# kyotovision-public/DRMNet

Measured on AMD Instinct MI355X. Metric: U-Net denoise steps/sec on 3x128x256 refmaps, higher is better.
Workload: dtype emulated fp32: f16 hi*hi + e4m3 cross terms (~15-bit products), fp32 acc; 1e-4 contract

## Files before the change

drmnet_amd/_lib.py:

```python
from __future__ import annotations

import ctypes as C
import os
from typing import Optional, Sequence

import torch

_HERE = os.path.dirname(os.path.abspath(__file__))
LIB_PATH = os.environ.get("DRM_LIB_PATH") or os.path.join(_HERE, "csrc", "libdrmnet_hip.so")
ABI_VERSION = 3
MAX_LEVELS = 8
LOSS_WORKSPACE_BYTES = 2048
DIFFUSION_LOSS_MAX_PARTS = 32


def diffusion_loss_workspace_bytes(B: int) -> int:
    return int(B) * DIFFUSION_LOSS_MAX_PARTS * 2 * 8


SYMBOLS = [
    "drm_abi_version", "drm_last_error",
    "drm_unet_create", "drm_unet_destroy", "drm_unet_param_count", "drm_unet_param_info", "drm_unet_load_params",
    "drm_unet_workspace_bytes", "drm_unet_forward",
    "drm_linear_forward", "drm_timestep_embedding", "drm_op_norm_act_conv", "drm_op_resblock", "drm_op_attention_block",
    "drm_drmnet_create", "drm_drmnet_destroy", "drm_drmnet_workspace_bytes", "drm_drmnet_set_batch_parts", "drm_drmnet_set_batch_part_min", "drm_drmnet_step", "drm_drmnet_sample",
    "drm_sampler_workspace_bytes", "drm_ddim_sample", "drm_ddim_sample_logged", "drm_ddpm_sample", "drm_ddim_sample_ex", "drm_ddpm_sample_ex", "drm_randn",
    "drm_profile_enable", "drm_profile_reset", "drm_profile_collect", "drm_unet_set_precision", "drm_set_op_precision",
    "drm_refmap_workspace_bytes", "drm_refmap_mask_make", "drm_erode_mask",
    "drm_unet_load_params_set", "drm_unet_use_set", "drm_set_graph_replay", "drm_set_upconv_split", "drm_graph_launches",
    "drm_map_chain", "drm_masked_log_range", "drm_luminance_scale", "drm_mirmap2envmap", "drm_hdr2ldr", "drm_resize", "drm_profile_variants",
    "drm_render_refmap", "drm_brdf_eval", "drm_render_refmap_views", "drm_validation_losses",
    "drm_render_refmap_lit", "drm_render_light_workspace_bytes",
    "drm_render_mesh_workspace_bytes", "drm_render_mesh",
    "drm_mesh_bvh_bytes", "drm_mesh_bvh_build", "drm_mesh_occluded", "drm_render_mesh_shadowed", "drm_render_mesh_lit",
    "drm_mesh_closest_hit", "drm_render_mesh_bounced",
    "drm_render_normals", "drm_image_from_refmap",
    "drm_obs_forward_process", "drm_diffusion_losses",
]


class UNetDesc(C.Structure):
    _fields_ = [
        ("kind", C.c_int32), ("in_channels", C.c_int32), ("model_channels", C.c_int32), ("out_channels", C.c_int32),
        ("num_res_blocks", C.c_int32), ("n_levels", C.c_int32), ("channel_mult", C.c_int32 * MAX_LEVELS),
# ... 116 lines not shown
    L.drm_ddpm_sample_ex.argtypes = [vp, fp, fp, fp, C.POINTER(C.c_float), i32, i32, fp, C.c_uint64, C.POINTER(SamplerOptions), i32, i32, i32, vp, C.c_size_t, vp]
    L.drm_randn.argtypes = [fp, C.c_size_t, C.c_uint64, C.c_uint64, vp]
    u8p = vp
    L.drm_refmap_workspace_bytes.argtypes = [C.c_int64, i32, C.c_float]
    L.drm_refmap_workspace_bytes.restype = C.c_size_t
    L.drm_refmap_mask_make.argtypes = [fp, fp, C.c_int64, i32, i32, C.c_float, i32, fp, u8p, vp, C.c_size_t, vp]
    L.drm_erode_mask.argtypes = [u8p, i32, i32, i32, u8p, vp]
    L.drm_unet_set_precision.argtypes = [vp, i32]
    L.drm_set_op_precision.argtypes = [i32]
    L.drm_profile_enable.argtypes = [i32]
    L.drm_profile_enable.restype = None
    L.drm_profile_reset.restype = None
    L.drm_profile_collect.argtypes = [C.POINTER(C.c_double), C.POINTER(C.c_double), C.POINTER(C.c_double), C.POINTER(C.c_int64)]
    L.drm_set_graph_replay.argtypes = [i32]
    L.drm_set_upconv_split.argtypes = [i32]
    L.drm_graph_launches.restype = C.c_int64
    L.drm_map_chain.argtypes = [fp, fp, C.c_int64, i32, C.POINTER(C.c_int32), C.POINTER(C.c_float), i32, fp, fp, fp, vp]
    L.drm_masked_log_range.argtypes = [fp, fp, i32, i32, i32, fp, fp, vp]
    L.drm_luminance_scale.argtypes = [fp, i32, i32, C.c_float, fp, vp]
    L.drm_mirmap2envmap.argtypes = [fp, fp, fp, i32, i32, i32, i32, i32, i32, i32, i32, vp]
    L.drm_hdr2ldr.argtypes = [fp, u8p, i32, C.c_float, C.c_float, fp, vp]
    L.drm_resize.argtypes = [fp, fp, i32, i32, i32, i32, i32, i32, vp]
    L.drm_profile_variants.argtypes = [C.c_char_p, C.c_size_t]
    L.drm_profile_variants.restype = C.c_size_t
    L.drm_render_refmap.argtypes = [fp, fp, fp, i32, i32, i32, i32, i32, i32, i32, vp]
    L.drm_brdf_eval.argtypes = [fp, i32, fp, fp, fp, fp, C.c_int64, vp]
    L.drm_render_refmap_views.argtypes = [fp, i32, fp, fp, fp, i32, i32, i32, i32, i32, i32, i32, vp]
    L.drm_render_refmap_lit.argtypes = [fp, i32, fp, fp, fp, i32, i32, i32, i32, i32, i32, i32, i32, vp, C.c_size_t, vp]
    L.drm_render_light_workspace_bytes.argtypes = [i32, i32, i32, i32]
    L.drm_render_light_workspace_bytes.restype = C.c_size_t
# ... 68 lines not shown
```

drmnet_amd/csrc/abi.hip:

```cpp
#include <atomic>
#include <cstring>
#include <memory>

#include "bvh.h"
#include "profiler.h"
#include "samplers.h"

using namespace drm;

struct drm_unet {
  UNet net;
};
struct drm_drmnet {
  DrmnetSampler s;
};

namespace {

int make_arena(Arena& ar, void* ws, size_t bytes, size_t need) {
  if (need == 0) return DRM_ERR_INVALID;
  if (bytes < need || ws == nullptr) {
    set_error("workspace too small: need " + std::to_string(need) + " bytes, got " + std::to_string(bytes));
    return DRM_ERR_WORKSPACE;
  }
// ... 409 lines not shown
    DRM_REQUIRE(precision_valid(precision),
                "precision must be 0 (fp32 MFMA), 1 (split fp16 x3), 2 (plain fp16 operands), 3 (split fp16 with fp8 cross terms) or 4 (plain bf16 operands)");
    g_op_precision.store(precision, std::memory_order_relaxed);
    return DRM_OK;
  });
}

int drm_set_upconv_split(int mode) {
  return guarded([&]() -> int {
    DRM_REQUIRE(mode >= 0 && mode <= 2, "upconv split mode: 0 = never, 1 = by the measured rule, 2 = wherever the form applies");
    set_upconv_split(mode);
    return DRM_OK;
  });
}

int drm_set_graph_replay(int on) {
  set_graph_replay(on != 0);
  return DRM_OK;
}
int64_t drm_graph_launches(void) { return (int64_t)graph_launches(); }

void drm_profile_enable(int on) { prof_enable(on); }
void drm_profile_reset(void) { prof_reset(); }
int drm_profile_collect(double* ms, double* flops, double* bytes, int64_t* launches) {
  return guarded([&]() -> int {
    DRM_REQUIRE(ms && flops && bytes && launches, "null argument");
    prof_collect(ms, flops, bytes, launches);
    return DRM_OK;
  });
}
// ... 220 lines not shown
```

drmnet_amd/csrc/common.h:

```cpp
#pragma once
#include <hip/hip_runtime.h>
#include <stdint.h>
#include <stdio.h>
#include <atomic>
#include <string>
#include "conv_forms.h"
#include "gn_fold.h"

namespace drm {

void set_error(const std::string& msg);
const char* last_error();

#define DRM_OK 0
#define DRM_ERR_INVALID 1
#define DRM_ERR_HIP 2
#define DRM_ERR_WORKSPACE 3
#define DRM_ERR_STATE 4

#define DRM_HIP_CHECK(expr)                                                                              \
  do {                                                                                                   \
    hipError_t _e = (expr);                                                                              \
    if (_e != hipSuccess) {                                                                              \
      ::drm::set_error(std::string(#expr) + " failed: " + hipGetErrorString(_e) + " at " + __FILE__ + ":" + \
// ... 66 lines not shown
  int terms = 3;
  int mx_site = 0;
#ifdef DRM_S2_STAMP
  unsigned* stamp_out = nullptr;
  int stamp_block = 0, stamp_tile0 = 0;
#endif
  double2* stat_out = nullptr;
  float* pool_out = nullptr;
  double2* pool_stat = nullptr;
  const float* w_inv_scale = nullptr;
  int ld0 = 0;
  int gn_ld = 0;
  long long w_img_stride_f4 = 0;
  const float* w_inv_img = nullptr;
  int prof_kind = -1;
  const float* in_inv = nullptr;
  GnFold gnf;
};
struct ConvWork { double flops, bytes; };
inline ConvWork conv_work(const ConvArgs& a, int taps) {
  const double cin = a.cin_real > 0 ? a.cin_real : (a.C0 + a.C1), cout = a.out_nchw ? a.cout_valid : a.Cout;
  const double px = (double)a.N * a.H * a.W;
  const double px_in = (double)a.N * ((a.H >> a.up0) * (a.W >> a.up0)) * a.C0 + px * a.C1;
  return {2.0 * px * (taps == 4 ? 9 : taps) * cin * cout, 4.0 * (px_in + px * cout * (a.res ? 2 : 1) + (double)taps * cin * cout)};
}
enum ConvKernel : unsigned char { CONV_NONE, CONV_IGEMM, CONV_PIPELINE };
enum SplitFinish : unsigned char { SPLIT_NONE, SPLIT_IN_LAUNCH, SPLIT_REDUCE };
struct ConvPlan {
  ConvKernel kernel = CONV_NONE;
  int terms = 0;
  ConvTile tile = TILE_128x32;
  int th = 0, tw = 0;
  bool ragged = false;
  int kc = 32;
  int ksplit = 1;
  SplitFinish finish = SPLIT_NONE;
  size_t tickets = 0;
  bool pool = false;
  bool gn_fold = false;
// ... 2 lines not shown
ConvPlan plan_conv(const ConvArgs& a, int precision, bool want_pool = false, bool gn_foldable = false);
bool conv_split_weights(int precision, int cin);
int launch_conv(const ConvArgs& a, const ConvPlan& p, hipStream_t s);
template <int TAPS, int TERMS> int dispatch_s2(const ConvArgs& a, const ConvPlan& p, hipStream_t s);
int no_form(const ConvPlan& p);
size_t packed_conv_weight_split_floats(int taps, int CoutP, int CinP);
int launch_pack_conv_weight_split(const float* w, float* packed, float* scales, unsigned* scratch, int Cout, int Cin, int taps, int CoutP,
                                  int CinP, hipStream_t s, bool mx = false, bool bf16 = false);
enum Precision { PREC_FP32 = 0, PREC_F16X3 = 1, PREC_F16 = 2, PREC_F16MX = 3, PREC_BF16 = 4 };
inline bool precision_valid(int p) { return p >= PREC_FP32 && p <= PREC_BF16; }
inline int precision_terms(int p) { return p == PREC_F16 ? 1 : (p == PREC_BF16 ? 4 : (p == PREC_FP32 ? 0 : 3)); }
int launch_pack_conv_weight(const float* w, float* packed, int Cout, int Cin, int taps, int CoutP, int CinP, hipStream_t s);
int pack_conv_image(int precision, const float* w, float* packed, float* scale, unsigned* scratch, int Cout, int Cin, int taps, int CoutP, int CinP,
                    bool mx_site, hipStream_t s);
int launch_fold_upconv_weight(const float* w, float* wa, float* wb, int Cout, int C0, int C1, hipStream_t s);
int launch_fold_attn_params(const float* qkv_w, const float* qkv_b, const float* proj_w, const float* proj_b, float* w_out, float* b_out, int C,
                            hipStream_t s);
size_t packed_conv_weight_floats(int taps, int CoutP, int CinP);

int launch_chan_moments(const float* x, int N, int HW, int C, double* partial , double2* mom , hipStream_t s);
int chan_moments_splits(int HW, int C);
int launch_act_pow2_scale(const double2* mom0, int C0, int lo0, int hi0, double cnt0, const double2* mom1, int C1, double cnt1,
                          const unsigned* absmax_bits, int Ctab, int N, float* scale, float* shift, float* inv, hipStream_t s, int absmax_parts = 1);
int launch_gn_finalize(const double2* mom0, int C0, double inv0, const double2* mom1, int C1, double inv1, const float* gamma,
                       const float* beta, int N, float* scale, float* shift, hipStream_t s, double cnt0 = 0.0, double cnt1 = 0.0,
                       float* guard_scale = nullptr, float* guard_shift = nullptr, float* guard_inv = nullptr);

size_t refmap_workspace_bytes(long long n, int res, float thr);
int launch_refmap_mask_make(const float* colors, const float* normals, long long n, int C, int res, float thr, int min_points, float* refmap,
                            unsigned char* refmask, void* ws, size_t ws_bytes, hipStream_t s);
// ... 106 lines not shown
```

drmnet_amd/csrc/conv.hip:

```cpp

#include "common.h"
#include "profiler.h"

namespace drm {

typedef float f32x16 __attribute__((ext_vector_type(16)));

template <int TAPS, int TH, int TW, int WM, int WN, int MT, int NT, int KC>
struct Cfg {
  static constexpr int BM = WM * MT * 32;
  static constexpr int BN = WN * NT * 32;
  static constexpr int TN = BM / (TH * TW);
  static constexpr int HALO = (TAPS == 9) ? 1 : 0;
  static constexpr int HT = TH + 2 * HALO, WT = TW + 2 * HALO;
  static constexpr int HPI = HT * WT;
  static constexpr int HP = TN * HPI;
  static constexpr int KG = KC / 4;
  static constexpr int TPI = 256 / TN;
  static constexpr int A_SLOTS = (HPI * KG + TPI - 1) / TPI;
  static constexpr int B_F4 = KG * BN;
  static constexpr int B_SLOTS = (B_F4 + 255) / 256;
  static constexpr int LDS_F4 = KG * HP + 2 * B_F4;
  static_assert(BM == 128 && WM * WN == 4, "4 waves, 128 GEMM rows");
  static_assert(KG % 2 == 0 && TPI % KG == 0, "k-group split across lane halves");
// ... 302 lines not shown
        *d = make_double2(d->x + a, d->y + c2);
      }
    }
  }
}

#define DRM_X(TAPS, TERMS) extern template int dispatch_s2<TAPS, TERMS>(const ConvArgs&, const ConvPlan&, hipStream_t);
DRM_S2_UNITS(DRM_X)
#undef DRM_X
int launch_conv(const ConvArgs& a, const ConvPlan& p, hipStream_t s) {
  DRM_REQUIRE(a.taps == 9 || a.taps == 1 || a.taps == 4, "conv taps must be 9, 1 or 4 (the parity form of a 3x3 over a nearest-x2 input)");
  DRM_REQUIRE(a.taps != 4 || (p.kernel == CONV_PIPELINE && p.finish == SPLIT_NONE), "the parity (4-tap) form runs on the pipeline kernel, un-split");
  DRM_REQUIRE(a.N > 0 && a.H > 0 && a.W > 0, "conv shape");
  DRM_REQUIRE(!a.up0 || (a.H % 2 == 0 && a.W % 2 == 0), "upsampled source needs even output size");
  DRM_REQUIRE(a.ksplit == p.ksplit && (p.ksplit == 1 || a.split_ws), "split-K launch without its slab workspace");
  if (p.kernel == CONV_IGEMM) return launch_igemm(a, p, s);
  DRM_REQUIRE(p.kernel == CONV_PIPELINE, "no conv kernel takes this shape (per-image weights: split modes, maps of whole 16x16 tiles, 128-channel multiples)");
  DRM_REQUIRE(a.Cout % 32 == 0 && (a.C0 + a.C1) % 32 == 0 && a.C0 % 32 == 0, "split conv needs channels % 32 == 0");
  DRM_REQUIRE(a.terms == p.terms, "ConvArgs::terms differs from the plan");
  DRM_REQUIRE(p.terms != 2 || (a.taps != 1 && a.gn_scale && !a.in_inv && a.w_img_stride_f4 == 0), "f16mx: 3x3 convs on a GroupNorm-ed input only");
  auto run = [&](const ConvArgs& x) -> int {
#define DRM_X(TAPS, TERMS) if (a.taps == TAPS && p.terms == TERMS) return dispatch_s2<TAPS, TERMS>(x, p, s);
    DRM_S2_UNITS(DRM_X)
#undef DRM_X
    return no_form(p);
  };
  if (p.finish != SPLIT_REDUCE) return run(a);
  ConvArgs part = a;
  part.out = a.split_ws;
  part.split_ws = nullptr;
// ... 38 lines not shown
```

drmnet_amd/csrc/conv_split.hip:

```cpp
#include "common.h"
#include "profiler.h"

namespace drm {

__global__ void absmax_kernel(const float* __restrict__ w, size_t n, unsigned* __restrict__ out_bits) {
  float m = 0.f;
  for (size_t i = blockIdx.x * (size_t)blockDim.x + threadIdx.x; i < n; i += (size_t)gridDim.x * blockDim.x) m = fmaxf(m, fabsf(w[i]));
#pragma unroll
  for (int o = 32; o > 0; o >>= 1) m = fmaxf(m, __shfl_xor(m, o));
  if ((threadIdx.x & 63) == 0) atomicMax(out_bits, __float_as_uint(m));
}

__global__ void split_scale_kernel(const unsigned* __restrict__ absmax_bits, float* __restrict__ scales) {
  const float m = __uint_as_float(*absmax_bits);
  int k = 0;
  if (m > 0.f && m < INFINITY) {
    int e;
    frexpf(m, &e);
    k = 14 - e;
    if (k > 30) k = 30;
    if (k < -30) k = -30;
  }
  scales[0] = ldexpf(1.0f, k);
  scales[1] = ldexpf(1.0f, -k);
// ... 128 lines not shown
      const int ci = t % C1;
      const int co = (int)(t / C1);
      wb[k] = w[((size_t)co * Cin + C0 + ci) * 9 + tap];
    }
  }
}

int launch_fold_upconv_weight(const float* w, float* wa, float* wb, int Cout, int C0, int C1, hipStream_t s) {
  DRM_REQUIRE(w && wa && wb && Cout > 0 && C0 > 0 && C1 > 0, "upsampled-conv weight fold: arguments");
  const size_t n = (size_t)16 * Cout * C0 + (size_t)Cout * C1 * 9;
  hipLaunchKernelGGL(fold_upconv_weight_kernel, dim3((unsigned)std::min<size_t>((n + 255) / 256, 4096)), dim3(256), 0, s, w, wa, wb, Cout, C0, C1);
  DRM_HIP_CHECK(hipGetLastError());
  return DRM_OK;
}

}
```

drmnet_amd/csrc/conv_split2.hip:

```cpp
#include <algorithm>
#include <utility>
#include <vector>
#include <cstdio>
#include <string>

#include "common.h"
#include "conv_epilogue.h"
#include "profiler.h"

#ifdef DRM_S2_STAMP
#define S2_STAMP(id)                                                                               \
  do {                                                                                             \
    if (stamp_on && stamp_n < 120) {                                                               \
      unsigned long long t_;                                                                       \
      __builtin_amdgcn_sched_barrier(0);                                                           \
      asm volatile("s_memtime %0\n\ts_waitcnt lgkmcnt(0)" : "=s"(t_)::"memory");                   \
      __builtin_amdgcn_sched_barrier(0);                                                           \
      if (lane == 0) {                                                                             \
        stamp_lds[(wave * 120 + stamp_n) * 2] = (unsigned)(id);                                    \
        stamp_lds[(wave * 120 + stamp_n) * 2 + 1] = (unsigned)t_;                                  \
      }                                                                                            \
      ++stamp_n;                                                                                   \
    }                                                                                              \
  } while (0)
// ... 203 lines not shown
  bool stamp_on = false;
  if (a.stamp_out && (int)blockIdx.x == (a.stamp_block & 0xFFFF))
    for (int k = tid; k < C::NW * 240; k += C::NTHR) stamp_lds[k] = 0;
  stamp_on = a.stamp_out && (int)blockIdx.x == (a.stamp_block & 0xFFFF) && a.stamp_tile0 == 0;
  S2_STAMP(60);
#endif

  const int Ctot = a.C0 + a.C1;
  const int nch_all = Ctot / C::KC;
  const int ks = a.ksplit > 1 ? a.ksplit : 1;
  const int split = blockIdx.y;
  const int chunk0 = split * nch_all / ks;
  const int nchunks = (split + 1) * nch_all / ks - chunk0;
  const int NGT = nchunks * C::NG;
  constexpr bool FUSE = SK;
  static_assert(!SK || (WM == 4 && WN == 1 && MT == 1 && NT == 1 && !RAG), "split-K launches use the 128-row x 32-channel tiles (plan_conv)");
  const bool fused = FUSE && ks > 1 && a.split_ws != nullptr;
  float* const out_s = (fused ? a.split_ws : a.out) + (size_t)split * a.split_stride;
  const bool has_gn = a.gn_scale != nullptr;

  const int l_img = tid / C::TPI;
  const int l_tid = tid % C::TPI;
  const int l_o = tid % C::OCT;
  f32x4 areg[C::A_SLOTS][2];
  f32x4 sc[2], sh[2];
  unsigned avalid = 0;

  auto load_A_piece = [&](const TilePos& tp, int chunk, int piece) {
    const int c = (chunk0 + chunk) * C::KC;
    const float* src;
// ... 596 lines not shown
        }
        S2_STAMP(20 + 4 * (i * NT + c));
        const bool first = ks == 1;
        const float bias = (a.bias && first) ? a.bias[co] : 0.f;
        float rv[16], ev[4], sv[4];
#pragma unroll
        for (int g = 0; g < 4; ++g) {
          ev[g] = (a.emb && first) ? a.emb[(size_t)nimg[g] * a.emb_stride + co] : 0.f;
          sv[g] = epi_scale(a, nimg[g], inv_scale);
        }
#ifdef DRM_S2_STAMP
        const bool abl_noload = a.stamp_block & 0x200000;
#else
        constexpr bool abl_noload = false;
#endif
        if (a.res && first && !abl_noload) {
#pragma unroll
          for (int e = 0; e < 16; ++e) rv[e] = a.res[(pixb[e >> 2] + (e & 3)) * a.Cout + co];
        } else {
#pragma unroll
          for (int e = 0; e < 16; ++e) rv[e] = 0.f;
        }
        float s0 = 0.f, q0 = 0.f, s1 = 0.f, q1 = 0.f;
        float v[16];
#pragma unroll
        for (int e = 0; e < 16; ++e) {
          const int g = e >> 2;
          v[e] = epi_value(acc[i][c][e] * sv[g], bias, ev[g], rv[e]);
          acc[i][c][e] = 0.f;
#ifdef DRM_S2_STAMP
          if (a.stamp_block & 0x100000) continue;
// ... 259 lines not shown
  if (a.stamp_out && (int)blockIdx.x == (a.stamp_block & 0xFFFF)) {
    asm volatile("s_waitcnt lgkmcnt(0)" ::: "memory");
    __builtin_amdgcn_s_barrier();
    for (int k = tid; k < C::NW * 240; k += C::NTHR) a.stamp_out[k] = stamp_lds[k];
  }
#endif
}

template <int TAPS, int TH, int TW, int WM, int WN, int MT, int NT, int R, int TPS, int TERMS = 3, bool RAG = false, bool SK = false, bool POOL = false>
static int launch_s2(const ConvArgs& a, hipStream_t s) {
  using C = S2Cfg<TAPS, TH, TW, WM, WN, MT, NT, R, TPS, TERMS>;
  constexpr auto kern = conv_split2_kernel<TAPS, TH, TW, WM, WN, MT, NT, R, TPS, TERMS, RAG, SK, POOL>;
  DRM_REQUIRE(RAG || (a.H % TH == 0 && a.W % TW == 0), "conv tile does not divide the map");
  DRM_REQUIRE(POOL == (a.pool_out != nullptr), "pooled output: only launches plan_conv pools");
  DRM_REQUIRE(!POOL || (a.pool_stat && a.stat_out && a.ksplit <= 1 && !a.out_nchw), "pooled output: needs both statistics tables, no split-K");
  if constexpr (TAPS == 4) {
    static_assert(!RAG && !SK && !POOL, "the parity form has no ragged, split-K or pooled instantiation");
    DRM_REQUIRE(!a.bias && !a.emb && !a.res && !a.stat_out && !a.out_nchw && a.ksplit <= 1 && !a.gnf.mom0 && !a.in_inv && a.w_img_stride_f4 == 0,
                "parity (4-tap) conv: weight un-scaling only -- no bias, emb, residual, statistics, split-K or GroupNorm fold");
    DRM_REQUIRE(a.C1 == 0 && !a.up0 && a.Cout % 4 == 0 && (a.Cout / 4) % C::BN == 0, "parity (4-tap) conv: one stored source, a Cout tile inside one parity");
  }
  const size_t lds_bytes = (size_t)(C::LDS_F4 + (POOL ? C::ST_F4 : 0)) * sizeof(float4);
  static_assert((C::LDS_F4 + (POOL ? C::ST_F4 : 0)) * 16 <= 160 * 1024, "LDS budget");
  const DeviceInfo* di = device_info();
  if (!di) return DRM_ERR_STATE;
  DRM_TRY(opt_in_lds<kern>(lds_bytes, di));
  const int groups = (a.N + C::TN - 1) / C::TN;
  const long long tiles = (long long)groups * ((a.H + TH - 1) / TH) * ((a.W + TW - 1) / TW) * (a.Cout / C::BN);
  DRM_REQUIRE(tiles > 0 && tiles < (1ll << 31), "conv grid size");
  const int per_cu = std::max(1, std::min((int)(di->lds_per_cu / lds_bytes), 8 / C::NW));
// ... 94 lines not shown
```

drmnet_amd/csrc/engine.h:

```cpp
#pragma once
#include <map>
#include <string>
#include <tuple>
#include <vector>

#include "../../include/drmnet_hip.h"
#include "common.h"

namespace drm {

struct Arena {
  char* base = nullptr;
  size_t cap = 0, off = 0, peak = 0;
  bool dry = false;
  bool failed = false;
  void* alloc_bytes(size_t bytes) {
    const size_t a = (off + 255) & ~size_t(255);
    off = a + bytes;
    if (off > peak) peak = off;
    if (dry) return nullptr;
    if (off > cap) {
      failed = true;
      return nullptr;
    }
// ... 63 lines not shown
  size_t scale_dst = 0;
  bool mx_site = false;
  bool attn_fold = false;
  int up_c0 = 0;
  size_t upa_dst = 0, upa_scale = 0, upb_dst = 0, upb_scale = 0;
};

struct ResLayer {
  int cin = 0, cout = 0;
  size_t n1_w = 0, n1_b = 0, c1_w = 0, c1_b = 0, n2_w = 0, n2_b = 0, c2_w = 0, c2_b = 0, sk_w = 0, sk_b = 0;
  size_t c1_s = 0, c2_s = 0, sk_s = 0;
  int emb_off = 0;
  bool has_skip = false;
  int up_c0 = 0;
  size_t c1a_w = 0, c1a_s = 0, c1b_w = 0, c1b_s = 0;
};
struct AttnLayer {
  int ch = 0;
  size_t n_w = 0, n_b = 0, qkv_w = 0, qkv_b = 0, qkv_s = 0;
};
struct Layer {
  enum Kind { RES, ATTN, DOWN, UP } kind;
  ResLayer res;
  AttnLayer attn;
};

struct ParamTable {
  std::vector<ParamSlot> params;
  int emb_dim = 0, emb_total = 0;
  size_t wbuf_floats = 0;
// ... 34 lines not shown
  int dry_forward(int N, int H, int W, Arena& probe);
  ~UNet();
};

struct Ctx {
  Arena* ar;
  hipStream_t s;
  int N;
  int precision = PREC_FP32;
  bool dry() const { return ar->dry; }
  bool split() const { return precision == PREC_F16X3 || precision == PREC_F16 || precision == PREC_F16MX || precision == PREC_BF16; }
  int terms() const { return precision_terms(precision); }
};
Act new_act(Ctx& c, int C, int H, int W);
void set_upconv_split(int mode);
inline bool upconv_split_packable(int c0, int c1, int cout) { return c0 > 0 && c1 > 0 && c0 % 32 == 0 && c1 % 32 == 0 && cout % 32 == 0; }
int ensure_moments(Ctx& c, Act& a);
int expect_raw_sums(Ctx& c, Act& a);
int run_resblock(Ctx& c, const float* wbuf, const ResLayer& r, Act& x0, Act* x1, const float* emb_all, int emb_stride, Act& out, Act* pool = nullptr,
                 bool* pooled = nullptr);
int run_attention(Ctx& c, const float* wbuf, const AttnLayer& a, Act& x, Act& out);
int run_conv(Ctx& c, ConvArgs& a, const ConvPlan& p, const float* wbuf, size_t scale_off, Act* stats_for = nullptr);
int raw_input_guard(Ctx& c, ConvArgs& a, const ConvPlan& p, Act* x0, int lo0, int hi0, Act* x1, const unsigned* absmax_bits, int Ctab, int absmax_parts = 1);
int gn_params(Ctx& c, Act& x0, Act* x1, const float* gamma, const float* beta, float* scale, float* shift, ConvArgs* guard_for = nullptr,
              ConvArgs* fold_into = nullptr);

}
```

drmnet_amd/csrc/engine.hip:

```cpp
#include "engine.h"

#include <algorithm>
#include <atomic>
#include <deque>
#include <mutex>

namespace drm {

static thread_local std::string g_err;
void set_error(const std::string& msg) { g_err = msg; }
const char* last_error() { return g_err.c_str(); }

const DeviceInfo* device_info() {
  constexpr int MAX_DEV = 64;
  static DeviceInfo info[MAX_DEV];
  static std::atomic<int> state[MAX_DEV];
  int dev = 0;
  if (hipGetDevice(&dev) != hipSuccess || dev < 0 || dev >= MAX_DEV) {
    set_error("device_info: no current HIP device");
    return nullptr;
  }
  int st = state[dev].load(std::memory_order_acquire);
  if (st == 0) {
    static std::mutex mu;
// ... 81 lines not shown
    p.upb_scale = r.c1b_s = reserve(64);
  }
  r.c1_b = add_copy(px + ".in_layers.2.bias", {cout});
  r.emb_off = emb_total;
  emb_total += cout;
  ParamSlot ew; ew.name = px + ".emb_layers.1.weight"; ew.shape = {cout, emb_dim}; ew.kind = PK_COPY; ew.count = (size_t)cout * emb_dim; ew.dst = (size_t)-1; ew.cout = r.emb_off;
  params.push_back(ew);
  ParamSlot eb; eb.name = px + ".emb_layers.1.bias"; eb.shape = {cout}; eb.kind = PK_COPY; eb.count = (size_t)cout; eb.dst = (size_t)-2; eb.cout = r.emb_off;
  params.push_back(eb);
  r.n2_w = add_copy(px + ".out_layers.0.weight", {cout});
  r.n2_b = add_copy(px + ".out_layers.0.bias", {cout});
  r.c2_w = add_conv(px + ".out_layers.3.weight", cout, cout, 3, cout, cout, false, &r.c2_s, true);
  r.c2_b = add_copy(px + ".out_layers.3.bias", {cout});
  if (r.has_skip) {
    r.sk_w = add_conv(px + ".skip_connection.weight", cout, cin, 1, cout, cin, false, &r.sk_s);
    r.sk_b = add_copy(px + ".skip_connection.bias", {cout});
  }
}

void ParamTable::add_attn(Layer& l, const std::string& px, int ch) {
  l.kind = Layer::ATTN;
  AttnLayer& a = l.attn;
  a.ch = ch;
  a.n_w = add_copy(px + ".norm.weight", {ch});
  a.n_b = add_copy(px + ".norm.bias", {ch});
  a.qkv_w = add_conv(px + ".qkv.weight", 3 * ch, ch, 1, 3 * ch, ch, true, &a.qkv_s);
  params.back().attn_fold = true;
  a.qkv_b = add_copy(px + ".qkv.bias", {3 * ch});
  params.back().kind = PK_FOLDED;
  ParamSlot pw; pw.name = px + ".proj_out.weight"; pw.shape = {ch, ch, 1}; pw.kind = PK_FOLDED; pw.count = (size_t)ch * ch;
// ... 114 lines not shown
  }
}

int pack_conv_image(int precision, const float* w, float* packed, float* scale, unsigned* scratch, int Cout, int Cin, int taps, int CoutP, int CinP,
                    bool mx_site, hipStream_t s) {
  if (conv_split_weights(precision, CinP))
    return launch_pack_conv_weight_split(w, packed, scale, scratch, Cout, Cin, taps, CoutP, CinP, s, precision == PREC_F16MX && mx_site,
                                         precision == PREC_BF16);
  return launch_pack_conv_weight(w, packed, Cout, Cin, taps, CoutP, CinP, s);
}

size_t ParamTable::staging_floats() const {
  size_t n = 0;
  for (const ParamSlot& p : params) {
    if (p.attn_fold) n = std::max(n, (size_t)p.cout * p.cin + (size_t)p.cout);
    if (p.up_c0) n = std::max(n, (size_t)16 * p.cout * p.up_c0 + (size_t)9 * p.cout * (p.cin - p.up_c0));
  }
  return n;
}

int ParamTable::pack(const float* const* ptrs, int count, float* wbuf, int precision, float* staging, hipStream_t s) const {
  DRM_REQUIRE(count == (int)params.size(), "parameter count mismatch: got " + std::to_string(count) + ", expected " + std::to_string(params.size()));
  DRM_HIP_CHECK(hipMemsetAsync(wbuf, 0, wbuf_floats * sizeof(float), s));
  auto conv = [&](const float* w, size_t dst, size_t scale_dst, int cout, int cin, int taps, int coutp, int cinp, bool mx_site) -> int {
    return pack_conv_image(precision, w, wbuf + dst, wbuf + scale_dst, reinterpret_cast<unsigned*>(wbuf + scratch_off), cout, cin, taps, coutp, cinp,
                           mx_site, s);
  };
  for (size_t i = 0; i < params.size(); ++i) {
    const ParamSlot& p = params[i];
    DRM_REQUIRE(ptrs[i] != nullptr, "null parameter pointer for " + p.name);
    if (p.kind == PK_FOLDED) continue;
    const float* w = ptrs[i];
    if (p.attn_fold) {
      DRM_REQUIRE(i + 3 < params.size() && ptrs[i + 1] && ptrs[i + 2] && ptrs[i + 3], "attention block parameters of " + p.name);
      float* fb = staging + (size_t)p.cout * p.cin;
      DRM_TRY(launch_fold_attn_params(ptrs[i], ptrs[i + 1], ptrs[i + 2], ptrs[i + 3], staging, fb, p.cin, s));
      DRM_HIP_CHECK(hipMemcpyAsync(wbuf + params[i + 1].dst, fb, (size_t)p.cout * sizeof(float), hipMemcpyDeviceToDevice, s));
      w = staging;
    }
    if (p.kind == PK_COPY) {
      DRM_HIP_CHECK(hipMemcpyAsync(wbuf + p.dst, w, p.count * sizeof(float), hipMemcpyDeviceToDevice, s));
    } else {
      DRM_TRY(conv(w, p.dst, p.scale_dst, p.cout, p.cin, p.taps, p.coutp, p.cinp, p.mx_site));
      if (p.up_c0) {
        const int c0 = p.up_c0, c1 = p.cin - p.up_c0;
        float* wa = staging;
        float* wb = staging + (size_t)16 * p.cout * c0;
        DRM_TRY(launch_fold_upconv_weight(w, wa, wb, p.cout, c0, c1, s));
        DRM_TRY(conv(wa, p.upa_dst, p.upa_scale, 4 * p.cout, c0, 4, 4 * p.cout, c0, p.mx_site));
        DRM_TRY(conv(wb, p.upb_dst, p.upb_scale, p.cout, c1, 9, p.cout, c1, p.mx_site));
      }
    }
  }
  return DRM_OK;
}

int UNet::load(const float* const* ptrs, int count, hipStream_t s, int set) {
  DRM_REQUIRE(set >= 0 && set < NSETS, "weight set index");
  if (!wsets[set]) DRM_HIP_CHECK(hipMalloc(reinterpret_cast<void**>(&wsets[set]), wbuf_floats * sizeof(float)));
// ... 117 lines not shown
  ConvPlan p4, p9;
};
static UpconvSplit plan_upconv_split(const Ctx& c, const ResLayer& r, const ConvArgs& a, const ConvPlan& pa, const Act& x0, const Act* x1) {
  UpconvSplit u;
  const int mode = g_upconv_split.load(std::memory_order_relaxed);
  if (mode == 0 || !r.up_c0 || !x0.up || !x1 || x0.C != r.up_c0 || !upconv_split_packable(x0.C, x1->C, r.cout)) return u;
  auto plain = [](const ConvPlan& p) { return p.kernel == CONV_PIPELINE && !p.ragged && p.ksplit == 1 && !p.gn_fold && !p.pool; };
  if (!plain(pa)) return u;
  u.a4.C0 = x0.C; u.a4.N = a.N; u.a4.H = a.H >> 1; u.a4.W = a.W >> 1; u.a4.taps = 4; u.a4.Cout = 4 * r.cout; u.a4.mx_site = 1;
  u.b9.C0 = x1->C; u.b9.N = a.N; u.b9.H = a.H; u.b9.W = a.W; u.b9.taps = 9; u.b9.Cout = r.cout; u.b9.mx_site = 1;
  u.p4 = plan_conv(u.a4, c.precision);
  u.p9 = plan_conv(u.b9, c.precision);
  if (!plain(u.p4) || !plain(u.p9)) return u;
  if (r.cout % tile_shape(u.p4.tile).bn() != 0) return u;
  if (mode == 1 && (u.p4.tile > TILE_256x128 || u.p9.tile > TILE_256x128)) return u;
  u.on = true;
  return u;
}

int run_resblock(Ctx& c, const float* Wb, const ResLayer& r, Act& x0, Act* x1, const float* emb_all, int emb_stride, Act& out, Act* pool, bool* pooled) {
  DRM_TRY(arena_ok(c));
  const int H = x0.H, W = x0.W;
  const int C0 = x0.C, C1 = x1 ? x1->C : 0;
  DRM_REQUIRE(C0 + C1 == r.cin, "resblock input channels");
  DRM_REQUIRE(!x1 || (x1->H == H && x1->W == W && !x1->up), "resblock skip tensor shape");
  DRM_REQUIRE(r.has_skip || (!x1 && !x0.up), "identity skip on a concatenated / upsampled input is not supported");
  const size_t mark = c.ar->mark();
  float* sc1 = c.ar->alloc<float>((size_t)c.N * r.cin);
  float* sh1 = c.ar->alloc<float>((size_t)c.N * r.cin);
  Act h1 = new_act(c, r.cout, H, W);
  float* sc2 = c.ar->alloc<float>((size_t)c.N * r.cout);
  float* sh2 = c.ar->alloc<float>((size_t)c.N * r.cout);
  ConvArgs k;
  ConvArgs a;
  a.src0 = x0.p; a.src1 = x1 ? x1->p : nullptr; a.C0 = C0; a.C1 = C1; a.up0 = x0.up;
  a.N = c.N; a.H = H; a.W = W; a.taps = 9; a.Cout = r.cout; a.mx_site = 1;
  const ConvPlan pa = plan_conv(a, c.precision, false, true);
  ConvPlan pk;
  if (r.has_skip) {
    k.C0 = C0; k.C1 = C1; k.N = c.N; k.H = H; k.W = W; k.taps = 1; k.Cout = r.cout;
    pk = plan_conv(k, c.precision);
  }
  DRM_TRY(gn_params(c, x0, x1, Wb + r.n1_w, Wb + r.n1_b, sc1, sh1, pk.split() ? &k : nullptr, pa.gn_fold ? &a : nullptr));
  splitk_workspace(c, a, pa);
  UpconvSplit up = plan_upconv_split(c, r, a, pa, x0, x1);
  if (up.on) {
    if (!c.dry()) {
      ConvArgs& a4 = up.a4;
      a4.src0 = x0.p; a4.gn_scale = sc1; a4.gn_shift = sh1; a4.gn_ld = r.cin; a4.silu = 1;
      a4.w = Wb + r.c1a_w; a4.out = h1.p;
      DRM_TRY(run_conv(c, a4, up.p4, Wb, r.c1a_s, nullptr));
      ConvArgs& b9 = up.b9;
      b9.src0 = x1->p; b9.gn_scale = sc1 + x0.C; b9.gn_shift = sh1 + x0.C; b9.gn_ld = r.cin; b9.silu = 1;
      b9.w = Wb + r.c1b_w; b9.bias = Wb + r.c1_b;
      b9.emb = emb_all ? emb_all + r.emb_off : nullptr; b9.emb_stride = emb_stride;
      b9.res = h1.p; b9.out = h1.p;
      DRM_TRY(run_conv(c, b9, up.p9, Wb, r.c1b_s, &h1));
    }
  } else if (!c.dry()) {
// ... 2 lines not shown
    a.emb = emb_all ? emb_all + r.emb_off : nullptr; a.emb_stride = emb_stride;
    a.out = h1.p;
    DRM_TRY(run_conv(c, a, pa, Wb, r.c1_s, &h1));
  }
  ConvArgs b;
  b.src0 = h1.p; b.C0 = r.cout; b.N = c.N; b.H = H; b.W = W; b.taps = 9; b.Cout = r.cout; b.mx_site = 1;
  const ConvPlan pb = plan_conv(b, c.precision, pool != nullptr, true);
  DRM_TRY(gn_params(c, h1, nullptr, Wb + r.n2_w, Wb + r.n2_b, sc2, sh2, nullptr, pb.gn_fold ? &b : nullptr));
  splitk_workspace(c, b, pb);
  if (pooled) *pooled = pb.pool;
  if (pb.pool) DRM_TRY(expect_raw_sums(c, *pool));
  if (r.has_skip) splitk_workspace(c, k, pk);
  if (!c.dry()) {
    const float* res = x0.p;
    if (r.has_skip) {
      k.src0 = x0.p; k.src1 = x1 ? x1->p : nullptr; k.up0 = x0.up;
      k.w = Wb + r.sk_w; k.bias = Wb + r.sk_b;
      k.out = out.p;
      DRM_TRY(run_conv(c, k, pk, Wb, r.sk_s, nullptr));
      res = out.p;
    }
    b.gn_scale = sc2; b.gn_shift = sh2; b.silu = 1;
    b.w = Wb + r.c2_w; b.bias = Wb + r.c2_b;
    b.res = res; b.out = out.p;
    if (pb.pool) {
      b.pool_out = pool->p;
      b.pool_stat = pool->mom;
    }
    DRM_TRY(run_conv(c, b, pb, Wb, r.c2_s, &out));
  }
  c.ar->release(mark);
  return DRM_OK;
}

// ... 222 lines not shown
```

drmnet_amd/ops.py:

```python
from __future__ import annotations

from typing import Optional, Sequence

import torch

from . import _lib


def set_precision(precision: str) -> None:
    modes = {"fp32": 0, "f16x3": 1, "f16": 2, "f16mx": 3, "bf16": 4}
    if precision not in modes:
        raise ValueError(f"precision must be one of {list(modes)}")
    _lib.check(_lib.lib().drm_set_op_precision(modes[precision]))


def set_graph_replay(on: bool) -> None:
    _lib.check(_lib.lib().drm_set_graph_replay(int(bool(on))))


def set_upconv_split(mode: int) -> None:
    _lib.check(_lib.lib().drm_set_upconv_split(int(mode)))


UPCONV_TAP_GROUPS = {0: {0: (0,), 1: (1, 2)}, 1: {0: (0, 1), 1: (2,)}}


def fold_upconv_weight(w: torch.Tensor, c0: int):
    cout = w.shape[0]
    w0 = w[:, :c0].double()
    wa = torch.zeros((4, cout, c0, 2, 2), dtype=torch.float64, device=w.device)
    for a in (0, 1):
        for b in (0, 1):
            for dy in (0, 1):
                for dx in (0, 1):
                    for ky in UPCONV_TAP_GROUPS[a][dy]:
                        for kx in UPCONV_TAP_GROUPS[b][dx]:
# ... 317 lines not shown
```

include/drmnet_hip.h:

```cpp
#ifndef DRMNET_HIP_H
#define DRMNET_HIP_H

#include <stddef.h>
#include <stdint.h>

#ifdef __cplusplus
extern "C" {
#endif

#define DRM_ABI_VERSION 3
#define DRM_MAX_LEVELS 8

int drm_abi_version(void);
const char* drm_last_error(void);

typedef struct drm_unet_desc {
  int32_t kind;
  int32_t in_channels;
  int32_t model_channels;
  int32_t out_channels;
  int32_t num_res_blocks;
  int32_t n_levels;
  int32_t channel_mult[DRM_MAX_LEVELS];
  int32_t n_attn;
// ... 87 lines not shown
  const float* dropout_keep;
} drm_sampler_options;

int drm_ddim_sample_ex(drm_unet* net, float* x, const float* cond, const int64_t* timesteps, const float* coef, int S, int num_steps,
                       const float* noise, uint64_t seed, const drm_sampler_options* opt, int log_every_t, float* log_x, float* log_pred_x0, int log_slots,
                       int32_t* n_logged, int N, int H, int W, void* workspace, size_t workspace_bytes, void* stream);
int drm_ddpm_sample_ex(drm_unet* net, float* x, float* pred_x0, const float* cond, const float* coef, int T_start, int clip_denoised,
                       const float* noise, uint64_t seed, const drm_sampler_options* opt, int N, int H, int W, void* workspace, size_t workspace_bytes,
                       void* stream);

size_t drm_sampler_workspace_bytes(const drm_unet* net, int N, int H, int W);

int drm_set_graph_replay(int on);

int drm_set_upconv_split(int mode);
int64_t drm_graph_launches(void);

#define DRM_PROFILE_KINDS 5
void drm_profile_enable(int on);
void drm_profile_reset(void);
int drm_profile_collect(double* ms, double* flops, double* bytes, int64_t* launches);
size_t drm_profile_variants(char* buf, size_t cap);

int drm_randn(float* out, size_t n, uint64_t seed, uint64_t offset, void* stream);

size_t drm_refmap_workspace_bytes(int64_t n, int res, float angle_threshold);
int drm_refmap_mask_make(const float* colors, const float* normals, int64_t n, int channels, int res, float angle_threshold, int min_points,
                         float* refmap, uint8_t* refmask, void* workspace, size_t workspace_bytes, void* stream);

int drm_erode_mask(const uint8_t* mask, int H, int W, int kernel_size, uint8_t* out, void* stream);
// ... 83 lines not shown
```

Before: 899.6.

## Commute 1x1 skip conv with nearest upsample in decoder resblocks

In decoder resblocks whose skip input concatenates an upsampled tensor with a full-resolution one, the 1x1 skip convolution is split by input channel. The upsampled part is convolved at half resolution, and the full-resolution part's conv reads that result back through a new upsampled-residual path. This cuts the skip conv's FLOPs and input traffic on the upsampled channels by about four times. The cost is an extra launch, extra packed weight slices, a new residual-load path in the pipeline kernel, and reuse of h1 as a temporary buffer.

```diff
diff --git a/drmnet_amd/_lib.py b/drmnet_amd/_lib.py
--- a/drmnet_amd/_lib.py
+++ b/drmnet_amd/_lib.py
@@ -27,7 +27,7 @@
     "drm_sampler_workspace_bytes", "drm_ddim_sample", "drm_ddim_sample_logged", "drm_ddpm_sample", "drm_ddim_sample_ex", "drm_ddpm_sample_ex", "drm_randn",
     "drm_profile_enable", "drm_profile_reset", "drm_profile_collect", "drm_unet_set_precision", "drm_set_op_precision",
     "drm_refmap_workspace_bytes", "drm_refmap_mask_make", "drm_erode_mask",
-    "drm_unet_load_params_set", "drm_unet_use_set", "drm_set_graph_replay", "drm_set_upconv_split", "drm_graph_launches",
+    "drm_unet_load_params_set", "drm_unet_use_set", "drm_set_graph_replay", "drm_set_upconv_split", "drm_set_skip_commute", "drm_graph_launches",
     "drm_map_chain", "drm_masked_log_range", "drm_luminance_scale", "drm_mirmap2envmap", "drm_hdr2ldr", "drm_resize", "drm_profile_variants",
     "drm_render_refmap", "drm_brdf_eval", "drm_render_refmap_views", "drm_validation_losses",
     "drm_render_refmap_lit", "drm_render_light_workspace_bytes",
@@ -174,6 +174,7 @@
     L.drm_profile_collect.argtypes = [C.POINTER(C.c_double), C.POINTER(C.c_double), C.POINTER(C.c_double), C.POINTER(C.c_int64)]
     L.drm_set_graph_replay.argtypes = [i32]
     L.drm_set_upconv_split.argtypes = [i32]
+    L.drm_set_skip_commute.argtypes = [i32]
     L.drm_graph_launches.restype = C.c_int64
     L.drm_map_chain.argtypes = [fp, fp, C.c_int64, i32, C.POINTER(C.c_int32), C.POINTER(C.c_float), i32, fp, fp, fp, vp]
     L.drm_masked_log_range.argtypes = [fp, fp, i32, i32, i32, fp, fp, vp]
diff --git a/drmnet_amd/csrc/abi.hip b/drmnet_amd/csrc/abi.hip
--- a/drmnet_amd/csrc/abi.hip
+++ b/drmnet_amd/csrc/abi.hip
@@ -447,6 +447,14 @@
   });
 }
 
+int drm_set_skip_commute(int mode) {
+  return guarded([&]() -> int {
+    DRM_REQUIRE(mode >= 0 && mode <= 2, "skip commute mode: 0 = never, 1 = by the measured rule, 2 = wherever the form applies");
+    set_skip_commute(mode);
+    return DRM_OK;
+  });
+}
+
 int drm_set_graph_replay(int on) {
   set_graph_replay(on != 0);
   return DRM_OK;
diff --git a/drmnet_amd/csrc/common.h b/drmnet_amd/csrc/common.h
--- a/drmnet_amd/csrc/common.h
+++ b/drmnet_amd/csrc/common.h
@@ -104,6 +104,7 @@
   long long w_img_stride_f4 = 0;
   const float* w_inv_img = nullptr;
   int prof_kind = -1;
+  int res_up = 0;
   const float* in_inv = nullptr;
   GnFold gnf;
 };
@@ -112,7 +113,7 @@
   const double cin = a.cin_real > 0 ? a.cin_real : (a.C0 + a.C1), cout = a.out_nchw ? a.cout_valid : a.Cout;
   const double px = (double)a.N * a.H * a.W;
   const double px_in = (double)a.N * ((a.H >> a.up0) * (a.W >> a.up0)) * a.C0 + px * a.C1;
-  return {2.0 * px * (taps == 4 ? 9 : taps) * cin * cout, 4.0 * (px_in + px * cout * (a.res ? 2 : 1) + (double)taps * cin * cout)};
+  return {2.0 * px * (taps == 4 ? 9 : taps) * cin * cout, 4.0 * (px_in + px * cout * (a.res ? (a.res_up ? 1.25 : 2) : 1) + (double)taps * cin * cout)};
 }
 enum ConvKernel : unsigned char { CONV_NONE, CONV_IGEMM, CONV_PIPELINE };
 enum SplitFinish : unsigned char { SPLIT_NONE, SPLIT_IN_LAUNCH, SPLIT_REDUCE };
@@ -145,6 +146,7 @@
 int pack_conv_image(int precision, const float* w, float* packed, float* scale, unsigned* scratch, int Cout, int Cin, int taps, int CoutP, int CinP,
                     bool mx_site, hipStream_t s);
 int launch_fold_upconv_weight(const float* w, float* wa, float* wb, int Cout, int C0, int C1, hipStream_t s);
+int launch_slice_conv1x1_weight(const float* w, float* wa, float* wb, int Cout, int C0, int C1, hipStream_t s);
 int launch_fold_attn_params(const float* qkv_w, const float* qkv_b, const float* proj_w, const float* proj_b, float* w_out, float* b_out, int C,
                             hipStream_t s);
 size_t packed_conv_weight_floats(int taps, int CoutP, int CinP);
diff --git a/drmnet_amd/csrc/conv.hip b/drmnet_amd/csrc/conv.hip
--- a/drmnet_amd/csrc/conv.hip
+++ b/drmnet_amd/csrc/conv.hip
@@ -340,6 +340,8 @@
   DRM_REQUIRE(a.N > 0 && a.H > 0 && a.W > 0, "conv shape");
   DRM_REQUIRE(!a.up0 || (a.H % 2 == 0 && a.W % 2 == 0), "upsampled source needs even output size");
   DRM_REQUIRE(a.ksplit == p.ksplit && (p.ksplit == 1 || a.split_ws), "split-K launch without its slab workspace");
+  DRM_REQUIRE(!a.res_up || (p.kernel == CONV_PIPELINE && a.taps == 1 && !p.ragged && p.ksplit == 1 && !p.pool),
+              "a residual read at half resolution (res_up) is taken by whole-tile, un-split 1x1 pipeline launches only");
   if (p.kernel == CONV_IGEMM) return launch_igemm(a, p, s);
   DRM_REQUIRE(p.kernel == CONV_PIPELINE, "no conv kernel takes this shape (per-image weights: split modes, maps of whole 16x16 tiles, 128-channel multiples)");
   DRM_REQUIRE(a.Cout % 32 == 0 && (a.C0 + a.C1) % 32 == 0 && a.C0 % 32 == 0, "split conv needs channels % 32 == 0");
diff --git a/drmnet_amd/csrc/conv_split.hip b/drmnet_amd/csrc/conv_split.hip
--- a/drmnet_amd/csrc/conv_split.hip
+++ b/drmnet_amd/csrc/conv_split.hip
@@ -166,4 +166,24 @@
   return DRM_OK;
 }
 
+__global__ __launch_bounds__(256) void slice_conv1x1_weight_kernel(const float* __restrict__ w, float* __restrict__ wa, float* __restrict__ wb, int Cout,
+                                                                   int C0, int C1) {
+  const int Cin = C0 + C1;
+  const size_t n = (size_t)Cout * Cin;
+  for (size_t i = blockIdx.x * (size_t)blockDim.x + threadIdx.x; i < n; i += (size_t)gridDim.x * blockDim.x) {
+    const int ci = i % Cin;
+    const size_t co = i / Cin;
+    if (ci < C0) wa[co * C0 + ci] = w[i];
+    else wb[co * C1 + (ci - C0)] = w[i];
+  }
 }
+
+int launch_slice_conv1x1_weight(const float* w, float* wa, float* wb, int Cout, int C0, int C1, hipStream_t s) {
+  DRM_REQUIRE(w && wa && wb && Cout > 0 && C0 > 0 && C1 > 0, "1x1 weight slices: arguments");
+  const size_t n = (size_t)Cout * (C0 + C1);
+  hipLaunchKernelGGL(slice_conv1x1_weight_kernel, dim3((unsigned)std::min<size_t>((n + 255) / 256, 4096)), dim3(256), 0, s, w, wa, wb, Cout, C0, C1);
+  DRM_HIP_CHECK(hipGetLastError());
+  return DRM_OK;
+}
+
+}
diff --git a/drmnet_amd/csrc/conv_split2.hip b/drmnet_amd/csrc/conv_split2.hip
--- a/drmnet_amd/csrc/conv_split2.hip
+++ b/drmnet_amd/csrc/conv_split2.hip
@@ -241,6 +241,7 @@
   const int nchunks = (split + 1) * nch_all / ks - chunk0;
   const int NGT = nchunks * C::NG;
   constexpr bool FUSE = SK;
+  constexpr bool RES_UP = TAPS == 1 && !RAG && !SK && !POOL;
   static_assert(!SK || (WM == 4 && WN == 1 && MT == 1 && NT == 1 && !RAG), "split-K launches use the 128-row x 32-channel tiles (plan_conv)");
   const bool fused = FUSE && ks > 1 && a.split_ws != nullptr;
   float* const out_s = (fused ? a.split_ws : a.out) + (size_t)split * a.split_stride;
@@ -867,7 +868,18 @@
 #else
         constexpr bool abl_noload = false;
 #endif
-        if (a.res && first && !abl_noload) {
+        if (RES_UP && a.res && a.res_up && first && !abl_noload) {
+          if constexpr (RES_UP) {
+#pragma unroll
+            for (int g = 0; g < 4; ++g) {
+              int img, py, px;
+              C::rowmap((wm * MT + i) * 32 + 8 * g + 4 * h, img, py, px);
+              const size_t pixu = ((size_t)nimg[g] * (a.H >> 1) + ((cur.ty0 + py) >> 1)) * (a.W >> 1) + ((cur.tx0 + px) >> 1);
+#pragma unroll
+              for (int k = 0; k < 4; ++k) rv[4 * g + k] = a.res[(pixu + (k >> 1)) * a.Cout + co];
+            }
+          }
+        } else if (a.res && first && !abl_noload) {
 #pragma unroll
           for (int e = 0; e < 16; ++e) rv[e] = a.res[(pixb[e >> 2] + (e & 3)) * a.Cout + co];
         } else {
@@ -1157,6 +1169,8 @@
   DRM_REQUIRE(RAG || (a.H % TH == 0 && a.W % TW == 0), "conv tile does not divide the map");
   DRM_REQUIRE(POOL == (a.pool_out != nullptr), "pooled output: only launches plan_conv pools");
   DRM_REQUIRE(!POOL || (a.pool_stat && a.stat_out && a.ksplit <= 1 && !a.out_nchw), "pooled output: needs both statistics tables, no split-K");
+  DRM_REQUIRE(!a.res_up || (TAPS == 1 && !RAG && !SK && !POOL && a.res && a.ksplit <= 1 && !a.out_nchw && a.H % 2 == 0 && a.W % 2 == 0),
+              "half-resolution residual (res_up): whole-tile, un-split 1x1 launches on an even map only");
   if constexpr (TAPS == 4) {
     static_assert(!RAG && !SK && !POOL, "the parity form has no ragged, split-K or pooled instantiation");
     DRM_REQUIRE(!a.bias && !a.emb && !a.res && !a.stat_out && !a.out_nchw && a.ksplit <= 1 && !a.gnf.mom0 && !a.in_inv && a.w_img_stride_f4 == 0,
diff --git a/drmnet_amd/csrc/engine.h b/drmnet_amd/csrc/engine.h
--- a/drmnet_amd/csrc/engine.h
+++ b/drmnet_amd/csrc/engine.h
@@ -101,6 +101,7 @@
   bool has_skip = false;
   int up_c0 = 0;
   size_t c1a_w = 0, c1a_s = 0, c1b_w = 0, c1b_s = 0;
+  size_t ska_w = 0, ska_s = 0, skb_w = 0, skb_s = 0;
 };
 struct AttnLayer {
   int ch = 0;
@@ -165,6 +166,7 @@
 };
 Act new_act(Ctx& c, int C, int H, int W);
 void set_upconv_split(int mode);
+void set_skip_commute(int mode);
 inline bool upconv_split_packable(int c0, int c1, int cout) { return c0 > 0 && c1 > 0 && c0 % 32 == 0 && c1 % 32 == 0 && cout % 32 == 0; }
 int ensure_moments(Ctx& c, Act& a);
 int expect_raw_sums(Ctx& c, Act& a);
diff --git a/drmnet_amd/csrc/engine.hip b/drmnet_amd/csrc/engine.hip
--- a/drmnet_amd/csrc/engine.hip
+++ b/drmnet_amd/csrc/engine.hip
@@ -119,6 +119,14 @@
   r.c2_b = add_copy(px + ".out_layers.3.bias", {cout});
   if (r.has_skip) {
     r.sk_w = add_conv(px + ".skip_connection.weight", cout, cin, 1, cout, cin, false, &r.sk_s);
+    if (r.up_c0) {
+      ParamSlot& p = params.back();
+      p.up_c0 = up_c0;
+      p.upa_dst = r.ska_w = reserve(packed_conv_weight_floats(1, cout, up_c0));
+      p.upa_scale = r.ska_s = reserve(64);
+      p.upb_dst = r.skb_w = reserve(packed_conv_weight_floats(1, cout, cin - up_c0));
+      p.upb_scale = r.skb_s = reserve(64);
+    }
     r.sk_b = add_copy(px + ".skip_connection.bias", {cout});
   }
 }
@@ -263,7 +271,8 @@
   size_t n = 0;
   for (const ParamSlot& p : params) {
     if (p.attn_fold) n = std::max(n, (size_t)p.cout * p.cin + (size_t)p.cout);
-    if (p.up_c0) n = std::max(n, (size_t)16 * p.cout * p.up_c0 + (size_t)9 * p.cout * (p.cin - p.up_c0));
+    if (p.up_c0 && p.taps == 9) n = std::max(n, (size_t)16 * p.cout * p.up_c0 + (size_t)9 * p.cout * (p.cin - p.up_c0));
+    if (p.up_c0 && p.taps == 1) n = std::max(n, (size_t)p.cout * p.cin);
   }
   return n;
 }
@@ -291,7 +300,14 @@
       DRM_HIP_CHECK(hipMemcpyAsync(wbuf + p.dst, w, p.count * sizeof(float), hipMemcpyDeviceToDevice, s));
     } else {
       DRM_TRY(conv(w, p.dst, p.scale_dst, p.cout, p.cin, p.taps, p.coutp, p.cinp, p.mx_site));
-      if (p.up_c0) {
+      if (p.up_c0 && p.taps == 1) {
+        const int c0 = p.up_c0, c1 = p.cin - p.up_c0;
+        float* wa = staging;
+        float* wb = staging + (size_t)p.cout * c0;
+        DRM_TRY(launch_slice_conv1x1_weight(w, wa, wb, p.cout, c0, c1, s));
+        DRM_TRY(conv(wa, p.upa_dst, p.upa_scale, p.cout, c0, 1, p.cout, c0, p.mx_site));
+        DRM_TRY(conv(wb, p.upb_dst, p.upb_scale, p.cout, c1, 1, p.cout, c1, p.mx_site));
+      } else if (p.up_c0) {
         const int c0 = p.up_c0, c1 = p.cin - p.up_c0;
         float* wa = staging;
         float* wb = staging + (size_t)16 * p.cout * c0;
@@ -439,6 +455,30 @@
   if (!plain(u.p4) || !plain(u.p9)) return u;
   if (r.cout % tile_shape(u.p4.tile).bn() != 0) return u;
   if (mode == 1 && (u.p4.tile > TILE_256x128 || u.p9.tile > TILE_256x128)) return u;
+  u.on = true;
+  return u;
+}
+
+static std::atomic<int> g_skip_commute{1};
+void set_skip_commute(int mode) { g_skip_commute.store(mode); }
+
+struct SkipCommute {
+  bool on = false;
+  ConvArgs ka, kb;
+  ConvPlan pa, pb;
+};
+static SkipCommute plan_skip_commute(const Ctx& c, const ResLayer& r, const ConvArgs& k, const ConvPlan& pk, const ConvPlan& p_in, const Act& x0, const Act* x1) {
+  SkipCommute u;
+  const int mode = g_skip_commute.load(std::memory_order_relaxed);
+  if (mode == 0 || !r.has_skip || !r.up_c0 || !x0.up || !x1 || x0.C != r.up_c0 || !upconv_split_packable(x0.C, x1->C, r.cout)) return u;
+  auto plain = [](const ConvPlan& p) { return p.kernel == CONV_PIPELINE && !p.ragged && p.ksplit == 1 && !p.gn_fold && !p.pool; };
+  if (!plain(pk) || p_in.gn_fold || k.H % 2 != 0 || k.W % 2 != 0) return u;
+  u.ka.C0 = x0.C; u.ka.N = k.N; u.ka.H = k.H >> 1; u.ka.W = k.W >> 1; u.ka.taps = 1; u.ka.Cout = r.cout;
+  u.kb.C0 = x1->C; u.kb.N = k.N; u.kb.H = k.H; u.kb.W = k.W; u.kb.taps = 1; u.kb.Cout = r.cout;
+  u.pa = plan_conv(u.ka, c.precision);
+  u.pb = plan_conv(u.kb, c.precision);
+  if (!plain(u.pa) || !plain(u.pb)) return u;
+  if (mode == 1 && (u.pa.tile > TILE_256x128 || u.pb.tile > TILE_256x128)) return u;
   u.on = true;
   return u;
 }
@@ -468,6 +508,20 @@
   }
   DRM_TRY(gn_params(c, x0, x1, Wb + r.n1_w, Wb + r.n1_b, sc1, sh1, pk.split() ? &k : nullptr, pa.gn_fold ? &a : nullptr));
   splitk_workspace(c, a, pa);
+  SkipCommute sk = plan_skip_commute(c, r, k, pk, pa, x0, x1);
+  if (sk.on && !c.dry()) {
+    float* tmp = h1.p;
+    ConvArgs& ka = sk.ka;
+    ka.src0 = x0.p; ka.gn_scale = k.gn_scale; ka.gn_shift = k.gn_shift; ka.gn_ld = r.cin; ka.in_inv = k.in_inv;
+    ka.w = Wb + r.ska_w; ka.out = tmp;
+    DRM_TRY(run_conv(c, ka, sk.pa, Wb, r.ska_s, nullptr));
+    ConvArgs& kb = sk.kb;
+    kb.src0 = x1->p; kb.gn_ld = r.cin; kb.in_inv = k.in_inv;
+    kb.gn_scale = k.gn_scale ? k.gn_scale + x0.C : nullptr; kb.gn_shift = k.gn_shift ? k.gn_shift + x0.C : nullptr;
+    kb.w = Wb + r.skb_w; kb.bias = Wb + r.sk_b;
+    kb.res = tmp; kb.res_up = 1; kb.out = out.p;
+    DRM_TRY(run_conv(c, kb, sk.pb, Wb, r.skb_s, nullptr));
+  }
   UpconvSplit up = plan_upconv_split(c, r, a, pa, x0, x1);
   if (up.on) {
     if (!c.dry()) {
@@ -500,10 +554,12 @@
   if (!c.dry()) {
     const float* res = x0.p;
     if (r.has_skip) {
-      k.src0 = x0.p; k.src1 = x1 ? x1->p : nullptr; k.up0 = x0.up;
-      k.w = Wb + r.sk_w; k.bias = Wb + r.sk_b;
-      k.out = out.p;
-      DRM_TRY(run_conv(c, k, pk, Wb, r.sk_s, nullptr));
+      if (!sk.on) {
+        k.src0 = x0.p; k.src1 = x1 ? x1->p : nullptr; k.up0 = x0.up;
+        k.w = Wb + r.sk_w; k.bias = Wb + r.sk_b;
+        k.out = out.p;
+        DRM_TRY(run_conv(c, k, pk, Wb, r.sk_s, nullptr));
+      }
       res = out.p;
     }
     b.gn_scale = sc2; b.gn_shift = sh2; b.silu = 1;
diff --git a/drmnet_amd/ops.py b/drmnet_amd/ops.py
--- a/drmnet_amd/ops.py
+++ b/drmnet_amd/ops.py
@@ -20,6 +20,10 @@
 
 def set_upconv_split(mode: int) -> None:
     _lib.check(_lib.lib().drm_set_upconv_split(int(mode)))
+
+
+def set_skip_commute(mode: int) -> None:
+    _lib.check(_lib.lib().drm_set_skip_commute(int(mode)))
 
 
 UPCONV_TAP_GROUPS = {0: {0: (0,), 1: (1, 2)}, 1: {0: (0, 1), 1: (2,)}}
diff --git a/include/drmnet_hip.h b/include/drmnet_hip.h
--- a/include/drmnet_hip.h
+++ b/include/drmnet_hip.h
@@ -125,6 +125,7 @@
 int drm_set_graph_replay(int on);
 
 int drm_set_upconv_split(int mode);
+int drm_set_skip_commute(int mode);
 int64_t drm_graph_launches(void);
 
 #define DRM_PROFILE_KINDS 5
```

New measurement: 902.4 (median of 6 runs). No clear change (+0.3%).
